# zyang1580/PDA

Measured on AMD Instinct MI355X. Metric: users/sec full-catalogue top-K@50 (eval), higher is better.
Workload: dtype f32; 1 GPU; C3: synthetic 1000000 users x 200000 items, d=128, PDA condition ((elu+1)*pop^0.22) head, masked top-K@50; ranks_seen=1

## Files before the change

__graft_entry__.py:

```python
import os
import subprocess
import sys

ROOT = os.path.dirname(os.path.abspath(__file__))
if ROOT not in sys.path:
    sys.path.insert(0, ROOT)


def build() -> None:
    subprocess.check_call(["make", "-C", os.path.join(ROOT, "pda_amd", "csrc"), "-j4"])
    subprocess.check_call(["make", "-C", os.path.join(ROOT, "oracle")])
    import pda_amd
    from pda_amd import _lib
    _lib.load()


def smoke() -> None:
    import numpy as np
    import torch
    from oracle import c_oracle, pda_oracle as po
    from pda_amd import ops

    assert torch.cuda.is_available(), "smoke() needs a GPU"
    dev = torch.device("cuda:0")
    rng = np.random.default_rng(2021)
    nU, nI, d, B, K = 700, 3000, 64, 512, 50
    U = (rng.standard_normal((nU, d)) * 0.1).astype(np.float32)
    I = (rng.standard_normal((nI, d)) * 0.1).astype(np.float32)
    pop = rng.uniform(0, 1, nI).astype(np.float32) ** 0.22
    hist = [np.unique(rng.integers(0, nI, rng.integers(0, 40))) for _ in range(nU)]
    users = np.arange(nU, dtype=np.int32)
    indptr = np.zeros(nU + 1, dtype=np.int64)
    indptr[1:] = np.cumsum([len(h) for h in hist])
    indices = np.concatenate(hist).astype(np.int32)

    h = ops.HistoryCSR(torch.from_numpy(indptr).to(dev), torch.from_numpy(indices).to(dev), by_user=True)
    idx, val = ops.recommend_topk(torch.from_numpy(U).to(dev), torch.from_numpy(I).to(dev),
                                  torch.from_numpy(users).to(dev), K, ops.HEAD_POP,
                                  torch.from_numpy(pop).to(dev), h)
    ridx, rval, sc = c_oracle.score_topk(U, I, users, K, 1, pop, indptr, indices, order=1, want_scores=True)
    np.testing.assert_allclose(val.cpu().numpy(), rval, rtol=2e-6, atol=1e-6)
    got = idx.cpu().numpy()
    agree = (got == ridx).mean()
    top = np.sort(np.where(np.isfinite(sc), sc, -np.inf), axis=1)[:, ::-1][:, :K + 1]
    gapped = np.min(top[:, :-1] - top[:, 1:], axis=1) > 1e-5
    assert gapped.sum() >= nU // 2, "smoke data should be mostly tie-free"
    np.testing.assert_array_equal(got[gapped], ridx[gapped])
    for r in np.nonzero(~gapped)[0]:
        for a, b in zip(got[r], ridx[r]):
            assert a == b or abs(sc[r, a] - sc[r, b]) <= 1e-5, (r, a, b)

    Ut, It = torch.from_numpy(U).to(dev), torch.from_numpy(I).to(dev)
    us = rng.permutation(nU)[:B].astype(np.int32)
    ps = rng.integers(0, nI, B).astype(np.int32)
    ng = rng.integers(0, nI, B).astype(np.int32)
    pp = pop[ps]
    pn = pop[ng]
    loss = torch.zeros(3, device=dev)
    ops.bpr_step(Ut, It, *(torch.from_numpy(x).to(dev) for x in (us, ps, ng, pp, pn)), regs=1e-2, reg_div=B,
                 lr=0.05, mode=ops.UPD_SGD_FUSED, loss_acc=loss)
    U1, I1, _, ref_loss = po.train_step(U, I, us, ps, ng, pp, pn, 1e-2, B, 0.05, optimizer="sgd")
    np.testing.assert_allclose(loss.cpu().numpy(), np.array(ref_loss), rtol=1e-5, atol=1e-6)
    np.testing.assert_allclose(Ut.cpu().numpy(), U1, atol=1e-6)
    np.testing.assert_allclose(It.cpu().numpy(), I1, atol=1e-6)
    torch.cuda.synchronize()
    print("smoke ok: eval agreement %.5f, loss %s" % (agree, loss.cpu().numpy()))


if __name__ == "__main__":
    build()
    if len(sys.argv) > 1 and sys.argv[1] == "smoke":
        smoke()
```

pda_amd/csrc/pda_score_topk_v4.hip:

```cpp
#include "pda_v4_shared.h"
#include <cstdlib>
#include <type_traits>

using namespace pda_topk;

namespace {

constexpr int kCap4 = 57;
constexpr int kRing4 = 128;
constexpr int kWarmTiles = 4;
constexpr int kMainWaves = 8;
#ifndef PDA_W4_ABL
#define PDA_W4_ABL 0
#endif
#ifndef PDA_V4_ABL
#define PDA_V4_ABL 0
#endif
#ifdef PDA_V4_PROF
__device__ unsigned long long pda_prof4[24];
#define PROF_T0(v) const long long v = __builtin_readcyclecounter()
#define PROF_T1(v, slot) prof[slot] += (unsigned long long)(__builtin_readcyclecounter() - v)
#define PROF_INC(slot, x) prof[slot] += (unsigned long long)(x)
#define PROF_FLUSH(first, last) do { if (lane == 0) for (int pq = (first); pq <= (last); ++pq) atomicAdd(&pda_prof4[pq], prof[pq]); } while (0)
#else
#define PROF_T0(v) do {} while (0)
#define PROF_T1(v, slot) do {} while (0)
#define PROF_INC(slot, x) do {} while (0)
#define PROF_FLUSH(first, last) do {} while (0)
#endif
constexpr unsigned kSpinMax = 1u << 26;


struct Args4 {
    const void* U;
    const void* I;
    const float* pop;
    const int32_t* users;
    const int64_t* hist_indptr;
    const int32_t* hist_indices;
    uint64_t* out_keys;
    const unsigned char* rows;
    const float* sufA;
    const float* sufB;
    const int* pos_of;
    unsigned* stats;
    uint64_t* lists_ws;
    int32_t* regroup_ws;
    float* pred_ws;
    const int32_t* row_perm;
    const uint32_t* hmask_ws;
    const uint32_t* bloom;
    const int* prep_hdr;
    const float* seed;
    int n_users_blk, item_offset, n_items_local, hist_row_mode, K, n_splits, n_tiles;
    int warm_tiles;
    int warm_sorted;
    uint64_t* handover;
    const unsigned char* rows5;
    const float* meta5;
    const unsigned char* ufrag;
    const float* unorm;
    int prep_hdr_pop;
    int warm_final;
    int warm_shared;
    float* seed_out;
    const int* n_users_dev;
    int lists_empty;
};


template <int D, bool BF>
__global__ void __launch_bounds__(256) prep4_kernel(const void* __restrict__ I, const float* __restrict__ pop, const int* __restrict__ order,
                                                    int n, int n_pad, unsigned char* __restrict__ rows, int* __restrict__ pos_of,
                                                    int* __restrict__ hdr, unsigned char* __restrict__ rows5, int* __restrict__ meta5, u32x4* __restrict__ pinfo,
                                                    int f16img) {
    constexpr int TPR = D / 8, RB = row_bytes(D);
    const int pos = blockIdx.x * (256 / TPR) + threadIdx.x / TPR, e = threadIdx.x % TPR;
    if (pos >= n_pad) return;
    unsigned char* rp = rows + (size_t)pos * RB;
    float ss = 0.f, popv = 1.0f, rs = 0.f;
    int src = -1;
    if (pos < n) {
        src = pos;
        if (order) {
            src = order[pos];
            if (src < 0 || src >= n) { if (e == 0) atomicOr(hdr, 1); src = 0; }
            else if (e == 0 && atomicExch(&pos_of[src], pos) != -1) atomicOr(hdr, 1);
        } else if (e == 0) {
            pos_of[pos] = pos;
        }
        if (pop) popv = pop[src];
        const f32x4 a = pda_load4<BF>(I, (size_t)src * D + 8 * e);
        const f32x4 b = pda_load4<BF>(I, (size_t)src * D + 8 * e + 4);
        u32x4 hq, lq;
        split8(a, b, hq, lq);
        *reinterpret_cast<u32x4*>(rp + 16 * e) = hq;
#pragma unroll
        for (int k = 0; k < 4; ++k) ss += a[k] * a[k] + b[k] * b[k];
        {
            const float pv = pop ? ((popv == popv) ? popv : 0.f) : 1.0f;
            f32x4 as = a, bs = b;
#pragma unroll
            for (int k = 0; k < 4; ++k) { as[k] *= pv; bs[k] *= pv; }
            u32x4 hs, ls;
            if (f16img) {
                hs = pack_half8(as, bs, rs);
            } else {
                split8(as, bs, hs, ls);
#pragma unroll
                for (int k = 0; k < 4; ++k) {
                    const float r0 = as[k] - __uint_as_float((k & 1) ? (hs[k >> 1] & 0xFFFF0000u) : (hs[k >> 1] << 16));
                    const float r1 = bs[k] - __uint_as_float((k & 1) ? (hs[2 + (k >> 1)] & 0xFFFF0000u) : (hs[2 + (k >> 1)] << 16));
                    rs += r0 * r0 + r1 * r1;
                }
            }
            const int r5 = pos & 31;
            const int sw = D >= 128 ? (r5 & 15) : ((r5 >> 1) & 7);
            *reinterpret_cast<u32x4*>(rows5 + (size_t)(pos >> 5) * (64 * D) + r5 * (2 * D) + ((e ^ sw) << 4)) = hs;
        }
    } else {
        const u32x4 z = {0u, 0u, 0u, 0u};
        *reinterpret_cast<u32x4*>(rp + 16 * e) = z;
        {
            const int r5 = pos & 31;
            const int sw = D >= 128 ? (r5 & 15) : ((r5 >> 1) & 7);
            *reinterpret_cast<u32x4*>(rows5 + (size_t)(pos >> 5) * (64 * D) + r5 * (2 * D) + ((e ^ sw) << 4)) = z;
        }
    }
#pragma unroll
    for (int o = TPR / 2; o > 0; o >>= 1) { ss += __shfl_xor(ss, o, 64); rs += __shfl_xor(rs, o, 64); }
    if (e == 0) {
        const float v = sqrtf(ss) * 1.0009765625f * 1.0001f;
        const float rv = sqrtf(rs) * 1.0009765625f * 1.0001f;
        {
            if (pos < n) {
                const float pv = pop ? ((popv == popv) ? popv : 0.f) : 1.0f;
                atomicMax(&meta5[4 * (pos >> 5)], __float_as_int(pop ? pv : 0.f));
                atomicMax(&meta5[4 * (pos >> 5) + 1], __float_as_int(pv * v * 1.000001f));
                atomicMax(&meta5[4 * (pos >> 5) + 2], __float_as_int(rv));
            }
        }
        uint32_t p1 = 0x3F80u, p2 = 0, p3 = 0, k1 = 0, k2 = 0;
        if (pop) {
            const float ip = (popv > 0.f) ? fminf((1.0f / popv) * 0.9999995f, 1.0e6f) : 1.0e6f;
            bf16_split3(ip, p1, p2, p3);
            k1 = 0x3F80u;
            k2 = bf16_up(8.0e-6f);
            if (!(popv == popv)) k1 = 0xFF61u;
        } else {
            k1 = bf16_up(8.0e-6f);
// ... 1594 lines not shown
    w.lists = al(pda_score_topk_workspace_bytes(n_users_blk));
    size_t b = w.lists;
    if (lists_in_hbm4(d)) {
        const size_t ut = 1024;
        b += ((size_t)n_users_blk + ut - 1) / ut * (size_t)n_splits * ut * kCap4 * 8 + 256;
    }
    w.bloom = al(b);
    w.hmask = al(w.bloom + (size_t)n_users_blk * 128);
    w.regroup = al(w.hmask + ((size_t)n_users_blk + kUserTile - 1) / kUserTile * (size_t)n_splits * kUserTile * 2 * kWarmTiles * 4);
    w.handover = al(w.regroup + (1024 + 4 * (size_t)n_users_blk) * 4);
    w.total = w.handover + (size_t)n_splits * (size_t)n_users_blk * kCap4 * 8;
    w.ufrag = al(w.total);
    w.unorm = w.ufrag;
    {
        const size_t n_pad = ((size_t)n_users_blk + kUT5 - 1) / kUT5 * kUT5;
        w.unorm = w.ufrag + al(n_pad * 2 * (size_t)d);
        w.total = w.unorm + al(n_pad * 4);
    }
    w.seed = w.total;
    w.total = w.seed + al((size_t)n_users_blk * 4);
    return w;
}
extern "C" size_t pda_score_topk4_workspace_bytes(int n_users_blk, int n_items_local, int d, int n_splits) {
    if (n_users_blk <= 0 || n_items_local <= 0 || (d != 64 && d != 128 && d != 256)) return 0;
    if (n_splits <= 0) n_splits = pda_score_topk4_auto_splits(n_users_blk, n_items_local, d);
    return ws4_layout(n_users_blk, d, n_splits).total;
}

int run_score4(const void* U, const void* I_shard, bool bf16, const void* prep, const float* pop_shard, const int32_t* users,
               int n_users_blk, int item_offset, int n_items_local, int d, const int64_t* hist_indptr, const int32_t* hist_indices,
               int hist_row_mode, int K, int head, int early_stop, int n_splits, uint64_t* out_keys, void* workspace, hipStream_t s,
               int phase = 3, const float* seed = nullptr, int warm_tiles = 0, const int* n_users_dev = nullptr) {
    if (!U || !I_shard || !prep || !users || !out_keys || !workspace) return PDA_ERR_ARG;
    if (n_users_blk <= 0 || n_items_local <= 0 || item_offset < 0) return PDA_ERR_ARG;
    if (K < 1 || K > PDA_MAX_K) return PDA_ERR_ARG;
    if (early_stop < 0 || (early_stop & ~0x7FF) != 0) return PDA_ERR_ARG;
    const bool warm_per_split = (early_stop & PDA_SWEEP_WARM_PER_SPLIT) != 0;
    int geometry = (early_stop & PDA_SWEEP_HUGE) ? 4 : (early_stop & PDA_SWEEP_MANY_CANDIDATES) ? 3 : 0;
    if (warm_tiles == 0) warm_tiles = (early_stop >> 4) & 7;
    early_stop &= 1;
    if (head != PDA_HEAD_RAW && head != PDA_HEAD_POP) return PDA_ERR_ARG;
    if (head == PDA_HEAD_POP && !pop_shard) return PDA_ERR_ARG;
    if (hist_indptr && !hist_indices) return PDA_ERR_ARG;
    if (d != 64 && d != 128 && d != 256) return PDA_ERR_UNSUPPORTED;
    if (K > kCap4 - 3) return PDA_ERR_UNSUPPORTED;
    if ((uint64_t)n_items_local > (1ull << 26)) return PDA_ERR_UNSUPPORTED;
    if (warm_tiles < 0 || warm_tiles > kWarmTiles) return PDA_ERR_ARG;
#ifndef PDA_V4_WARM_DEFAULT
#define PDA_V4_WARM_DEFAULT kWarmTiles
#endif
    if (warm_tiles == 0) warm_tiles = d <= 128 ? PDA_V4_WARM_DEFAULT : kWarmTiles;
    const bool from_empty = phase == 4;
    if (from_empty) {
        if (seed == nullptr) return PDA_ERR_ARG;
        phase = 2;
        warm_tiles = 0;
    } else if (phase < 1 || phase > 3) {
        return PDA_ERR_ARG;
    }
    if (n_splits <= 0) n_splits = pda_score_topk4_auto_splits(n_users_blk, n_items_local, d);
    const Prep4Layout L = prep4_layout(n_items_local, d);
    const unsigned char* pb = reinterpret_cast<const unsigned char*>(prep);
    if (((phase & 1) || from_empty) && hipMemsetAsync(workspace, 0, pda_score_topk_workspace_bytes(n_users_blk), s) != hipSuccess) return PDA_ERR_LAUNCH;
    const Ws4 W = ws4_layout(n_users_blk, d, n_splits);
    unsigned char* wsb = reinterpret_cast<unsigned char*>(workspace);
    const float* sA = reinterpret_cast<const float*>(pb + (head == PDA_HEAD_POP ? L.sufA : L.sufB));
    const float* sB = reinterpret_cast<const float*>(pb + (head == PDA_HEAD_POP ? L.sufB : L.sufR));
    Args4 g{U, I_shard, pop_shard, users, hist_indptr, hist_indices, out_keys, pb + L.rows,
            early_stop ? sA : nullptr, early_stop ? sB : nullptr, reinterpret_cast<const int*>(pb + L.pos_of),
            reinterpret_cast<unsigned*>(workspace), reinterpret_cast<uint64_t*>(wsb + W.lists), nullptr, nullptr, nullptr, nullptr, nullptr, reinterpret_cast<const int*>(pb + L.hdr), seed, n_users_blk, item_offset, n_items_local, hist_row_mode, K, n_splits, L.n_tiles, warm_tiles,
#ifdef PDA_V4_WARM_SORTED
            1, nullptr, pb + L.rows5, reinterpret_cast<const float*>(pb + L.meta5), nullptr, nullptr, 0};
#else
            (phase == 1 || (L.n_tiles + n_splits - 1) / n_splits <= warm_tiles) ? 1 : 0, nullptr,
            pb + L.rows5, reinterpret_cast<const float*>(pb + L.meta5), nullptr, nullptr, 0};
#endif
    if (phase == 3 && !g.warm_sorted && PDA_V4_HANDOVER_WS) g.handover = reinterpret_cast<uint64_t*>(wsb + W.handover);
    g.ufrag = wsb + W.ufrag;
    g.unorm = reinterpret_cast<const float*>(wsb + W.unorm);
    g.prep_hdr_pop = (head == PDA_HEAD_POP && pop_shard != nullptr) ? 1 : 0;
    g.warm_final = (geometry >= 4 && phase == 3 && g.handover != nullptr && g.prep_hdr_pop && !early_stop) ? 1 : 0;
    g.lists_empty = from_empty ? 1 : 0;
    g.n_users_dev = n_users_dev;
    if (phase == 3 && n_splits > 1 && seed == nullptr && !warm_per_split && L.n_tiles > n_splits * warm_tiles) {
        g.warm_shared = 1;
        g.seed_out = reinterpret_cast<float*>(wsb + W.seed);
    }
    if (hist_indptr && (phase & 2)) {
        uint32_t* bloom = reinterpret_cast<uint32_t*>(wsb + W.bloom);
        hipLaunchKernelGGL(hist_bloom4_kernel, dim3((unsigned)((n_users_blk + 31) / 32)), dim3(256), 0, s, users, hist_indptr, hist_indices,
                           hist_row_mode, n_users_blk, bloom, reinterpret_cast<const int*>(pb + L.hdr), head == PDA_HEAD_POP ? 1 : 0);
        PDA_CHECK_LAUNCH();
        g.bloom = bloom;
    }
    if (hist_indptr && (phase & 1) && n_users_blk >= 98304) {
        uint32_t* hm = reinterpret_cast<uint32_t*>(wsb + W.hmask);
        const int utiles = (n_users_blk + kUserTile - 1) / kUserTile;
        Args4 gm = g;
        if (g.warm_shared) {
            gm.n_splits = 1;
            gm.warm_shared = 0;
        }
        hipLaunchKernelGGL(warm_mask4_kernel, dim3((unsigned)(utiles * gm.n_splits)), dim3(kThreads), 0, s, gm, hm);
        PDA_CHECK_LAUNCH();
        g.hmask_ws = hm;
    }
#ifndef PDA_V4_REGROUP_MIN
#define PDA_V4_REGROUP_MIN 98304
#endif
    if (early_stop && (phase & 2) && n_splits == 1 && n_users_blk >= PDA_V4_REGROUP_MIN) {
        g.regroup_ws = reinterpret_cast<int32_t*>(wsb + W.regroup);
        if (phase & 1) g.pred_ws = reinterpret_cast<float*>(g.regroup_ws + 1024 + 2 * (size_t)n_users_blk);
    }
    if (head == PDA_HEAD_RAW) {
        g.sufA = early_stop ? reinterpret_cast<const float*>(pb + L.sufA) : nullptr;
        g.sufB = early_stop ? reinterpret_cast<const float*>(pb + L.sufR) : nullptr;
    }
#define PDA_V4_(DD, BFV) (head == PDA_HEAD_POP ? launch4<DD, PDA_HEAD_POP, BFV>(g, phase, s, geometry) : launch4<DD, PDA_HEAD_RAW, BFV>(g, phase, s, geometry))
    switch (d) {
        case 64: return bf16 ? PDA_V4_(64, true) : PDA_V4_(64, false);
        case 128: return bf16 ? PDA_V4_(128, true) : PDA_V4_(128, false);
        case 256: return bf16 ? PDA_V4_(256, true) : PDA_V4_(256, false);
        default: return PDA_ERR_UNSUPPORTED;
    }
#undef PDA_V4_
}

__global__ void __launch_bounds__(256) kth_value_kernel(const uint64_t* __restrict__ keys, int S, int n_users, int K, int pos, float* __restrict__ out) {
    const int u = blockIdx.x * 256 + threadIdx.x;
    if (u >= n_users) return;
    float best = -INFINITY;
    for (int sp = 0; sp < S; ++sp) {
        const uint64_t k = keys[((size_t)sp * n_users + u) * K + pos];
        if (k != 0ull) best = fmaxf(best, pda_key_val(k));
    }
    out[u] = best;
}

__global__ void __launch_bounds__(256) seed_refine_kernel(const uint64_t* __restrict__ keys, int S, int n_users, int K, float* __restrict__ lo,
                                                          float* __restrict__ hi, float* __restrict__ mid, int32_t* __restrict__ counts, int mode) {
    const int u = blockIdx.x * 256 + threadIdx.x;
    if (u >= n_users) return;
    float l = lo[u], h = hi[u];
    if (mode >= 1) {
        if (counts[u] >= K) l = mid[u];
        else h = mid[u];
        lo[u] = l;
        hi[u] = h;
    }
    if (mode <= 1) {
        const bool open = l > -INFINITY && h < INFINITY && h > l;
        const float m = open ? l + 0.5f * (h - l) : l;
        int c = 0;
        for (int sp = 0; sp < S; ++sp) {
            const uint64_t* row = keys + ((size_t)sp * n_users + u) * K;
            for (int q = 0; q < K; ++q) {
                const uint64_t k = row[q];
                if (k == 0ull || pda_key_val(k) < m) break;
                ++c;
            }
        }
        mid[u] = m;
        counts[u] = c;
    }
}

// ... 193 lines not shown
```

pda_amd/csrc/pda_v5_sweep.h:

```cpp
#pragma once
#ifdef PDA_V6_LOOP_HEADER
#include PDA_V6_LOOP_HEADER
#else
#include "pda_v6_loop_asm.h"
#endif

#ifdef PDA_V5_LOG
__device__ unsigned pda_v5_log[1 << 18];
#define V5LOG(kind, a, b) do { if (lane == 0) { const unsigned i_ = atomicAdd(&pda_v5_log[0], 1u); if (i_ < (1u << 16) - 1u) { \
    pda_v5_log[4 * i_ + 4] = ((unsigned)blockIdx.x << 8) | (unsigned)wave; pda_v5_log[4 * i_ + 5] = (kind); pda_v5_log[4 * i_ + 6] = (a); pda_v5_log[4 * i_ + 7] = (b); } } } while (0)
#else
#define V5LOG(kind, a, b) do {} while (0)
#endif
constexpr int kRing5 = 192;



template <int D, bool BF, bool S16, int UPW>
__global__ void __launch_bounds__(256, 1) sweep5_kernel(Args4 g) {
    [[maybe_unused]] constexpr int HB = half_bytes5(D);
    static_assert(slot_bytes5(D) == Loop6<D, 8>::kSlotBytes, "one LDS image for all loops");
    static_assert(S16, "the loop on v_mfma_f32_32x32x16_bf16 (round 4's first form: 9.16 against 8.07 ms, profiles/README.md) left with round 5; the parameter keeps the kernel's name");
    static_assert((D <= 128 && UPW == 256) || (D == 256 && UPW == 128), "users per wave: 256, or (d = 256) 128 -- 8 blocks x 8 k-steps = 256 AGPRs, one 512-user workgroup per CU");
    constexpr int NK = D / 32, UBW = 16, NU = UPW / UBW;
    constexpr int SS = slot_bytes5(D), UT = 4 * UPW, CAPL = kCap4, RB4 = row_bytes(D);
    constexpr int LPC = D / 32, CPP = 64 / LPC;
    constexpr float kEps5 = BF ? 4.0234375e-3f : 8.046875e-3f;
    extern __shared__ __attribute__((aligned(16))) unsigned char smem[];
    unsigned char* tiles = smem;
    int* cntl = reinterpret_cast<int*>(smem + kNSlot5 * SS);
    float* taul = reinterpret_cast<float*>(cntl + UT);
    uint64_t* crings = reinterpret_cast<uint64_t*>(taul + UT);
    unsigned* sync = reinterpret_cast<unsigned*>(crings + 4 * kRing5);
    unsigned* s_uns = sync + 8;
    unsigned* touched = sync + 40;
    const int tid = threadIdx.x, lane = tid & 63;
    const int wave = __builtin_amdgcn_readfirstlane(tid >> 6);
    const int split = blockIdx.x % g.n_splits, utile = blockIdx.x / g.n_splits;
    uint64_t* lists = g.handover != nullptr ? g.handover + ((size_t)split * g.n_users_blk + (size_t)utile * UT) * kCap4
                                            : g.lists_ws + (size_t)blockIdx.x * UT * CAPL;
    const int K = g.K;
    const int nt = split_tiles(g.n_tiles, split, g.n_splits);
    const int wt = warm_tiles_of(g, split);
    const bool starts_empty = g.lists_empty || (g.warm_shared && split > 0);
    const bool warm_final = g.warm_final && !starts_empty;
    const int n_it = max(0, nt - wt);
    const unsigned hend = 2u * (unsigned)n_it;
    if (tid < 72) sync[tid] = (tid < 8 || tid >= 40 || warm_final || starts_empty) ? 0u : 0xFFFFFFFFu;
    if (tid == 0 && blockIdx.x == 0) g.stats[4] = (4u << 28) | (4u << 8) | (1u << 13) | ((BF ? 1u : 0u) << 14) | (unsigned)(D >> 6);
    if (starts_empty) {
        for (int rr = tid; rr < UT; rr += 256) {
            cntl[rr] = 0;
            taul[rr] = utile * UT + rr < g.n_users_blk ? -INFINITY : INFINITY;
        }
        __builtin_amdgcn_fence(__ATOMIC_RELEASE, "workgroup");
    } else if (warm_final) {
        for (int rr = tid; rr < UT; rr += 256) {
            const int rb = utile * UT + rr;
            int c = 0;
            float tau = INFINITY;
            if (rb < g.n_users_blk) {
                const uint64_t kl = lists[(size_t)rr * CAPL + (K - 1)];
                c = K;
                tau = pda_unordf((uint32_t)(kl >> 32));
                if (kl == 0ull) {
                    tau = -INFINITY;
                    for (c = 0; c < K - 1 && lists[(size_t)rr * CAPL + c] != 0ull; ++c) {}
                }
            }
            cntl[rr] = c;
            taul[rr] = tau;
        }
        __builtin_amdgcn_fence(__ATOMIC_RELEASE, "workgroup");
    } else
    {
        constexpr int NW = 4, PB = 8;
        for (int r0 = wave; r0 < UT; r0 += PB * NW) {
            uint64_t keyv[PB];
#pragma unroll
            for (int q = 0; q < PB; ++q) {
                const int rr = r0 + q * NW, rb = utile * UT + rr;
                keyv[q] = (rr >= UT || rb >= g.n_users_blk) ? 0ull
                          : g.handover != nullptr ? (lane < kCap4 ? g.handover[((size_t)split * g.n_users_blk + rb) * kCap4 + lane] : 0ull)
                          : (lane < K ? g.out_keys[((size_t)split * g.n_users_blk + rb) * K + lane] : 0ull);
            }
#pragma unroll
            for (int q = 0; q < PB; ++q) {
                const int rr = r0 + q * NW;
                if (rr >= UT) break;
                const int rb = utile * UT + rr;
                const uint64_t key = keyv[q];
                const int c = __popcll(__ballot(key != 0ull));
                if (g.handover == nullptr && lane < K) lists[(size_t)rr * CAPL + lane] = key;
                uint32_t mn = key != 0ull ? (uint32_t)(key >> 32) : 0xFFFFFFFFu;
#pragma unroll
                for (int o = 32; o >= 1; o >>= 1) mn = min(mn, (uint32_t)__shfl_xor((int)mn, o, 64));
                if (lane == 0) {
                    cntl[rr] = c;
                    taul[rr] = rb < g.n_users_blk ? (c >= K ? pda_unordf(mn) : -INFINITY) : INFINITY;
                }
            }
        }
        __builtin_amdgcn_fence(__ATOMIC_RELEASE, "workgroup");
    }
    __syncthreads();

    unsigned n_cand = 0;
    if (hend > 0) {
        const int row0 = wave * UPW;
        const int j = lane & (UBW - 1), hh = lane / UBW;
        const unsigned lane16 = (unsigned)lane * 16u;
        const unsigned char* my_ufrag = g.ufrag + ((size_t)utile * 4 + wave) * (size_t)(NU * NK * 1024);
        float eu = 0.f, seedv[NU];
#pragma unroll
        for (int u = 0; u < NU; ++u) {
            const int rb = utile * UT + row0 + UBW * u + j;
            eu = fmaxf(eu, rb < g.n_users_blk ? g.unorm[rb] : 0.f);
            seedv[u] = (g.seed != nullptr && rb < g.n_users_blk) ? g.seed[rb] : -INFINITY;
        }
#pragma unroll
        for (int o = 32; o >= 1; o >>= 1) eu = fmaxf(eu, __shfl_xor(eu, o, 64));
        eu = __int_as_float(__builtin_amdgcn_readfirstlane(__float_as_int(eu * (kEps5 * 1.001f))));
        const unsigned ring_lds = (unsigned)(size_t)(__attribute__((address_space(3))) unsigned char*)tiles;
        const unsigned flags_lds = (unsigned)(size_t)(__attribute__((address_space(3))) unsigned char*)reinterpret_cast<unsigned char*>(sync);
        uint64_t* my_ring = crings + wave * kRing5;
        unsigned ring_n = 0;
        const unsigned t0 = (unsigned)(split + wt * g.n_splits);
        const size_t img = (size_t)g.rows5, meta = (size_t)g.meta5;
        const bool hist_on = g.hist_indptr != nullptr;

        auto thr_of = [&](int u) __attribute__((always_inline)) -> float {
            const float tq = fmaxf(taul[row0 + UBW * u + j], seedv[u]);
            float tf = (tq == INFINITY || tq == -INFINITY) ? tq : tq - fabsf(tq) * 1.52587890625e-5f - 1e-30f;
            return fminf(fmaxf(tf, -1.0e30f), 1.0e30f);
        };
        auto rescore_ring = [&]() __attribute__((always_inline)) {
            const int q = lane % LPC, ci = lane / LPC;
            for (unsigned base = 0; base < ring_n; base += CPP) {
                const bool have = base + (unsigned)ci < ring_n;
                const uint64_t e = have ? my_ring[base + ci] : 0ull;
                const int row = (int)(e >> 32);
                const unsigned pos = (unsigned)e;
                bool valid = have && pos < (unsigned)g.n_items_local;
                const unsigned char* tail = g.rows + (size_t)(valid ? pos : 0u) * RB4 + 2 * D + 32;
                const float pv = *reinterpret_cast<const float*>(tail);
                const int loc = *reinterpret_cast<const int*>(tail + 4);
                const int rb = utile * UT + row0 + row;
                valid = valid && rb < g.n_users_blk;
                const int uid = valid ? g.users[rb] : 0;
                const float c_sd = (g.seed != nullptr && valid) ? g.seed[rb] : -INFINITY;
                const float c_tau = taul[row0 + (valid ? row : 0)];
                f32x4 uu[8], ii[8];
                const size_t ub = (size_t)uid * D + q * (LPC == 8 ? 32 : 8), ib = (size_t)(valid ? loc : 0) * D + q * (LPC == 8 ? 32 : 8);
#pragma unroll
                for (int c = 0; c < 8; ++c) {
                    const int off = LPC == 8 ? 4 * c : 8 * LPC * (c >> 1) + 4 * (c & 1);
                    uu[c] = pda_load4<BF>(g.U, ub + off);
                    ii[c] = pda_load4<BF>(g.I, ib + off);
                }
                long long hb = 0, he = 0;
                if (hist_on && valid) {
                    const int64_t hr = g.hist_row_mode == PDA_HIST_BY_USER_ID ? (int64_t)uid : (int64_t)rb;
                    hb = g.hist_indptr[hr];
                    he = g.hist_indptr[hr + 1];
                }
                auto fma8 = [&](float acc, int cq) __attribute__((always_inline)) -> float {
#pragma unroll
                    for (int sidx = 0; sidx < 4; ++sidx) {
                        acc = __builtin_fmaf(uu[2 * cq][sidx], ii[2 * cq][sidx], acc);
                        acc = __builtin_fmaf(uu[2 * cq + 1][sidx], ii[2 * cq + 1][sidx], acc);
                    }
                    return acc;
                };
                float o = 0.f, o_other = 0.f;
                if constexpr (LPC == 8) {
                    float c0 = 0.f, c1 = 0.f, o0 = 0.f, o1 = 0.f;
#pragma unroll
                    for (int ph = 0; ph < LPC; ++ph) {
                        o0 = c0;
                        o1 = c1;
#pragma unroll
                        for (int cc = 0; cc < 4; ++cc) {
#pragma unroll
                            for (int sidx = 0; sidx < 4; ++sidx) {
                                if (cc & 1) {
                                    o1 = __builtin_fmaf(uu[2 * cc][sidx], ii[2 * cc][sidx], o1);
                                    o1 = __builtin_fmaf(uu[2 * cc + 1][sidx], ii[2 * cc + 1][sidx], o1);
                                } else {
                                    o0 = __builtin_fmaf(uu[2 * cc][sidx], ii[2 * cc][sidx], o0);
                                    o0 = __builtin_fmaf(uu[2 * cc + 1][sidx], ii[2 * cc + 1][sidx], o0);
                                }
                            }
                        }
                        if (ph < LPC - 1) {
                            const float r0 = __shfl_up(o0, 1, 64), r1 = __shfl_up(o1, 1, 64);
                            if (q == ph + 1) {
                                c0 = r0;
                                c1 = r1;
                            }
                        }
                    }
                    o = o1;
                    o_other = o0;
                } else if constexpr (LPC == 4) {
// ... 6 lines not shown
                        const float a = fma8(o, cq);
                        const float a_sw = swap2(a);
                        const float b = fma8(hi ? a_sw : o, cq);
                        const float b_sw = swap2(b);
                        o = hi ? b : b_sw;
                    }
                } else {
                    static_assert(LPC == 2, "d = 64");
#pragma unroll
                    for (int cq = 0; cq < 4; ++cq) o = fma8(o, cq);
                }
                const float o0 = LPC == 8 ? o_other : __int_as_float(__builtin_amdgcn_mov_dpp(__float_as_int(o), 0xB1, 0xF, 0xF, true));
                float sc = o0 + o;
                sc = (sc > 0.0f ? sc + 1.0f : __expf(sc)) * pv;
                const float tt = (valid && q == LPC - 1) ? sc : -INFINITY;
                const int item = g.item_offset + loc;
                bool p = valid && q == LPC - 1 && (tt >= fmaxf(c_tau, c_sd));
                if (hist_on && p) {
                    long long lo = hb, hi2 = he;
                    while (lo < hi2) {
                        const long long mid = (lo + hi2) >> 1;
                        if (g.hist_indices[mid] < item) lo = mid + 1; else hi2 = mid;
                    }
                    if (lo < he && g.hist_indices[lo] == item) p = false;
                }
                const uint64_t key = pda_pack_key(tt, (uint32_t)item);
                if (p) atomicOr(&touched[(row0 + row) >> 5], 1u << ((row0 + row) & 31));
                append_keys<CAPL, true>(p, row0 + row, tt, key, lists, cntl, taul, row0, UPW, K, lane, s_uns);
            }
            n_cand += ring_n;
            ring_n = 0;
        };
        auto extract = [&](unsigned ft) __attribute__((always_inline)) {
            const unsigned T = t0 + (ft >> 1) * (unsigned)g.n_splits;
            const unsigned pos0 = T * 64u + (ft & 1u) * 32u;
            const float2 mt = *reinterpret_cast<const float2*>(g.meta5 + 4 * (size_t)(2u * T + (ft & 1u)));
            const float ct = __builtin_fmaf(eu, mt.y, mt.x);
            const unsigned char* tb = tiles + (ft & (kNSlot5 - 1)) * SS + j * (2 * D);
            auto item_of = [&](int r) __attribute__((always_inline)) -> unsigned {
                return 16u * (r >> 2) + 4u * hh + (r & 3);
            };
            constexpr int NR = 8;
            u32x4 af[2 * NK];
#pragma unroll
            for (int ib = 0; ib < 2; ++ib)
#pragma unroll
                for (int k = 0; k < NK; ++k) af[ib * NK + k] = *reinterpret_cast<const u32x4*>(tb + ib * 16 * (2 * D) + (((4 * k + hh) ^ swz5<D>(j)) << 4));
            for (int u = 0; u < NU; ++u) {
                const float tl = thr_of(u);
                const bool clampy = mt.x > tl;
                uint32_t m = 0;
#pragma unroll
                for (int ib = 0; ib < 2; ++ib) {
                    f32x4 acc = {0.f, 0.f, 0.f, 0.f};
#pragma unroll
                    for (int k = 0; k < NK; ++k) {
                        const u32x4 bf = *reinterpret_cast<const u32x4*>(my_ufrag + (((size_t)u * NK + k) * 64 + lane) * 16);
                        acc = __builtin_amdgcn_mfma_f32_16x16x32_bf16(__builtin_bit_cast(bf16x8, af[ib * NK + k]), __builtin_bit_cast(bf16x8, bf), acc, 0, 0, 0);
                    }
#pragma unroll
                    for (int r = 0; r < 4; ++r) m |= (acc[r] + ct > tl) ? (1u << (4 * ib + r)) : 0u;
                }
                if (__any(clampy)) {
#pragma unroll
                    for (int r = 0; r < NR; ++r) {
                        const unsigned pp = pos0 + item_of(r);
                        const float pi = clampy ? *reinterpret_cast<const float*>(g.rows + (size_t)pp * RB4 + 2 * D + 32) : 0.f;
                        m |= (clampy && pi > tl) ? (1u << r) : 0u;
                    }
                }
                while (__any(m != 0u)) {
                    if (ring_n + 64u > (unsigned)kRing5) rescore_ring();
                    const bool act = m != 0u;
                    const int r = __builtin_ctz(m | 0x10000u);
                    m &= ~(1u << r);
                    const uint64_t pm = __ballot(act);
                    const unsigned slot = ring_n + (unsigned)__builtin_amdgcn_mbcnt_hi((uint32_t)(pm >> 32), __builtin_amdgcn_mbcnt_lo((uint32_t)pm, 0));
                    if (act) my_ring[slot] = ((uint64_t)(unsigned)(UBW * u + j) << 32) | (uint64_t)(pos0 + item_of(r));
                    ring_n += (unsigned)__popcll(pm);
                }
            }
        };

        unsigned h = 0, issued = 0, n_entries = 0;
        bool hend_ok = true;
        if ((ring_lds & (D == 256 ? 511u : 255u)) != 0u) { if (lane == 0) g.stats[0] = 6u; hend_ok = false; }
        for (unsigned guard = 0; hend_ok && guard < 2u * hend + 8u; ++guard) {
            ++n_entries;
            float thr[NU];
#pragma unroll
            for (int u = 0; u < NU; ++u) thr[u] = thr_of(u);
            unsigned reason = 0;
            float tmin = thr[0];
#pragma unroll
            for (int u = 1; u < NU; ++u) tmin = fminf(tmin, thr[u]);
#pragma unroll
            for (int o = 32; o >= 1; o >>= 1) tmin = fminf(tmin, __shfl_xor(tmin, o, 64));
            tmin = __int_as_float(__builtin_amdgcn_readfirstlane(__float_as_int(tmin)));
            Loop6<D, NU>::run(h, issued, reason, hend, ring_lds, flags_lds, 1024u * (unsigned)wave, t0, (unsigned)g.n_splits,
                              (unsigned)img, (unsigned)(img >> 32), (unsigned)meta, (unsigned)(meta >> 32), eu, tmin, my_ufrag, thr, lane16);
            V5LOG(reason, h, issued);
            if (reason == 0u) break;
            if (reason != 1u) { if (lane == 0) g.stats[0] = 5u; break; }
#ifdef PDA_V5_LOG
            for (unsigned tq = (h >= 2u ? h - 2u : 0u); tq <= h && tq < hend; ++tq) {
                const unsigned Tq = t0 + (tq >> 1) * (unsigned)g.n_splits;
                const unsigned char* gsrc = g.rows5 + ((size_t)(2u * Tq + (tq & 1u))) * HB;
                const unsigned char* lsrc = tiles + (tq & (kNSlot5 - 1)) * SS;
                unsigned pieces = 0;
                for (int i = 0; i < HB / 1024; ++i) {
                    const u32x4 a4 = *reinterpret_cast<const u32x4*>(gsrc + i * 1024 + lane * 16);
                    const u32x4 b4 = *reinterpret_cast<const u32x4*>(lsrc + i * 1024 + lane * 16);
                    if (__ballot(((a4[0] ^ b4[0]) | (a4[1] ^ b4[1]) | (a4[2] ^ b4[2]) | (a4[3] ^ b4[3])) != 0u) != 0ull) pieces |= 1u << i;
                }
                if (pieces != 0u) V5LOG(13u, (tq << 8) | (h - tq), pieces);
            }
#endif
            [[maybe_unused]] const unsigned before = ring_n + n_cand;
            if (h >= 2u && h - 2u < hend) extract(h - 2u);
            if (h >= 1u && h - 1u < hend) extract(h - 1u);
            V5LOG(10u, h, ring_n + n_cand - before);
            if (ring_n >= (unsigned)CPP) rescore_ring();
        }
        if (ring_n > 0u) rescore_ring();
        if (lane == 0) atomicAdd(g.stats + 1, n_cand);
        if (lane == 0) atomicAdd(g.stats + 5, n_entries);
        if (lane == 0 && wave == 0) atomicAdd(reinterpret_cast<unsigned long long*>(g.stats + 2), (unsigned long long)(2 * n_it * (UT / kUserTile)));
    }
    __builtin_amdgcn_fence(__ATOMIC_ACQ_REL, "workgroup");
    __syncthreads();
    {
        constexpr int EB = 8;
        uint64_t* scr = crings + wave * kRing5;
        auto emit_row = [&](int rb, int cnt, uint64_t kraw) __attribute__((always_inline)) {
            const int c = min(__builtin_amdgcn_readfirstlane(cnt), CAPL);
            const uint64_t key = lane < c ? kraw : (uint64_t)(63 - lane);
            scr[lane] = key;
            pda_wave_sync();
            int rank = 0;
            for (int jj = 0; jj < c; jj += 4) {
                const uint64_t k0 = scr[jj], k1 = scr[jj + 1], k2 = scr[jj + 2], k3 = scr[jj + 3];
                rank += ((k0 > key) ? 1 : 0) + ((k1 > key) ? 1 : 0) + ((k2 > key) ? 1 : 0) + ((k3 > key) ? 1 : 0);
            }
            pda_wave_sync();
            uint64_t* orow = g.out_keys + ((size_t)split * g.n_users_blk + rb) * K;
            if (lane < c && rank < K) orow[rank] = key;
            if (lane >= c && lane < K) orow[lane] = 0ull;
        };
        if (warm_final) {
            for (int w = 0; w < UPW / 32; ++w) {
                unsigned m = touched[wave * (UPW / 32) + w];
                while (m != 0u) {
                    const int b = __builtin_ctz(m);
                    m &= m - 1u;
                    const int rr = wave * UPW + 32 * w + b;
                    emit_row(utile * UT + rr, cntl[rr], lists[(size_t)rr * CAPL + (lane < CAPL ? lane : CAPL - 1)]);
                }
            }
        } else if (starts_empty) {
            const int rb0 = utile * UT + wave * UPW, nv = max(0, min(UPW, g.n_users_blk - rb0));
            uint64_t* ob = g.out_keys + ((size_t)split * g.n_users_blk + rb0) * K;
            for (int i = lane; i < nv * K; i += 64) ob[i] = 0ull;
            __builtin_amdgcn_fence(__ATOMIC_RELEASE, "workgroup");
            for (int w = 0; w < UPW / 32; ++w) {
                unsigned m = touched[wave * (UPW / 32) + w];
                while (m != 0u) {
                    const int b = __builtin_ctz(m);
                    m &= m - 1u;
                    const int rr = wave * UPW + 32 * w + b;
                    emit_row(utile * UT + rr, cntl[rr], lists[(size_t)rr * CAPL + (lane < CAPL ? lane : CAPL - 1)]);
                }
            }
        } else {
            for (int i0 = 0; i0 < UPW; i0 += EB) {
                uint64_t kraw[EB];
                int cv[EB];
#pragma unroll
                for (int q = 0; q < EB; ++q) {
                    const int rr = wave * UPW + i0 + q, rb = utile * UT + rr;
                    const bool ok = rb < g.n_users_blk;
                    kraw[q] = ok ? lists[(size_t)rr * CAPL + (lane < CAPL ? lane : CAPL - 1)] : 0ull;
                    cv[q] = ok ? cntl[rr] : 0;
                }
#pragma unroll
                for (int q = 0; q < EB; ++q) {
                    const int rb = utile * UT + wave * UPW + i0 + q;
                    if (rb >= g.n_users_blk) break;
                    emit_row(rb, cv[q], kraw[q]);
                }
            }
        }
    }
}

template <int D, bool BF, bool S16, int UPW>
int launch_sweep5(const Args4& g, hipStream_t stream) {
    constexpr int UT = 4 * UPW;
    constexpr size_t lds = (size_t)kNSlot5 * slot_bytes5(D) + (size_t)UT * 8 + 4 * kRing5 * 8 + 80 * 4 + 64;
    static_assert(UPW == 256 || D == 256 || 2 * lds <= 160 * 1024, "two workgroups per CU");
    static_assert(lds <= 160 * 1024, "LDS per workgroup");
    static int attr_set = 0;
    if (!attr_set) {
        if (hipFuncSetAttribute(reinterpret_cast<const void*>(&sweep5_kernel<D, BF, S16, UPW>), hipFuncAttributeMaxDynamicSharedMemorySize, (int)lds) != hipSuccess)
            return PDA_ERR_LAUNCH;
        attr_set = 1;
    }
    const int utiles = (g.n_users_blk + UT - 1) / UT, n_pad = utiles * UT;
    hipLaunchKernelGGL((uprep5_kernel<D, BF, S16, UPW>), dim3((unsigned)(((size_t)n_pad * (D / 8) + 255) / 256)), dim3(256), 0, stream, g.U, g.users, g.n_users_blk, n_pad,
                       const_cast<unsigned char*>(g.ufrag), const_cast<float*>(g.unorm));
// ... 6 lines not shown
```

pda_amd/ops.py:

```python
from __future__ import annotations

import math
import os
from typing import Optional, Tuple

import ctypes as C

import torch

from . import _lib
from ._lib import (HEAD_POP, HEAD_RAW, HIST_BY_BLOCK_ROW, HIST_BY_USER_ID, UPD_ANY_ORDER, UPD_DENSE_GRAD, UPD_NONE, UPD_USERS_DISTINCT,
                   UPD_SGD_FUSED, check, ptr, stream_ptr)

ADAM_BETA1, ADAM_BETA2, ADAM_EPS = 0.9, 0.999, 1e-8


def _need(t: Optional[torch.Tensor], dtype, name: str, optional=False):
    if t is None:
        if optional:
            return None
        raise ValueError(f"{name} is required")
    if not t.is_cuda:
        raise ValueError(f"{name} must live in HBM (cuda tensor); pda_amd has no CPU path")
    if t.dtype != dtype:
# ... 323 lines not shown
    if pop_shard is not None and pop_shard.numel() != nloc:
        raise ValueError("pop_shard must have one entry per local item row")
    if nloc > (1 << 26):
        raise ValueError("seeded item-sharded evaluation: at most 2^26 item rows per shard")
    if head == HEAD_POP and pop_shard is not None:
        _check_pop(pop_shard)
    if hist is not None and hist.indices.numel() == 0:
        hist = None
    c = SeededCall()
    order = visiting_order(I_shard, pop_shard if head == HEAD_POP else None)
    prep = item_prep4(I_shard, pop_shard if head == HEAD_POP else None, order)
    if n_splits <= 0:
        n_splits = lib.pda_score_topk4_auto_splits(nu, nloc, d)
    c.lib, c.K, c.nu, c.n_splits, c.nloc, c.stats = lib, K, nu, n_splits, nloc, stats
    c.out = torch.empty((n_splits, nu, K), dtype=torch.int64, device=U.device)
    c.ws = torch.empty(lib.pda_score_topk4_workspace_bytes(nu, nloc, d, n_splits), dtype=torch.uint8, device=U.device)
    c.fnp = lib.pda_score_topk4_phase_bf16 if bf else lib.pda_score_topk4_phase_f32
    c.common = (ptr(U), ptr(I_shard), ptr(prep), ptr(pop_shard), ptr(users), nu, item_offset, nloc, d,
                ptr(hist.indptr) if hist else None, ptr(hist.indices) if hist else None, hist.mode if hist else 0, K, head,
                1 | few_candidates_hint(head, True, nu, d), n_splits)
    c.keep = (U, I_shard, prep, pop_shard, users, hist)
    c.wt = int(os.environ.get("PDA_WARM_TILES", "0")) or max(1, 4 // max(1, seed_shards))
    check(c.fnp(*c.common, 1, c.wt, None, ptr(c.out), ptr(c.ws), stream_ptr()), "pda_score_topk4_phase (warm-up)")
    c.bounds = torch.empty((3, nu), dtype=torch.float32, device=U.device)
    m = -(-K // max(1, seed_shards))
    check(lib.pda_topk_seed_bounds(ptr(c.out), n_splits, nu, K, m, ptr(c.bounds), stream_ptr()), "pda_topk_seed_bounds")
    c.n_thr, c.counts = seed_thresholds(seed_shards), None
    return c


def kth_value(keys: torch.Tensor, pos: int) -> torch.Tensor:
    keys = _need(keys, torch.int64, "keys")
    S, nu, K = keys.shape
    out = torch.empty(nu, dtype=torch.float32, device=keys.device)
    check(_lib.load().pda_topk_kth_value(ptr(keys), S, nu, K, int(pos), ptr(out), stream_ptr()), "pda_topk_kth_value")
    return out


def remap_key_items(keys: torch.Tensor, gid: torch.Tensor) -> torch.Tensor:
    keys = _need(keys, torch.int64, "keys")
    gid = _need(gid, torch.int32, "gid")
    check(_lib.load().pda_topk_remap_items(ptr(keys), keys.numel(), ptr(gid), gid.numel(), stream_ptr()), "pda_topk_remap_items")
    return keys


def sweep_from_seed(U, I_shard, users, K, head, pop_shard, hist, item_offset, seed: torch.Tensor, n_splits: int = 0, prune="order",
                    stats: Optional[dict] = None) -> torch.Tensor:
    lib = _lib.load()
    bf = I_shard.dtype == torch.bfloat16
    U = _need(U, torch.bfloat16 if bf else torch.float32, "U")
    I_shard = _need(I_shard, torch.bfloat16 if bf else torch.float32, "I_shard")
    users = _need(users, torch.int32, "users")
    seed = _need(seed, torch.float32, "seed")
    pop_shard = _need(pop_shard, torch.float32, "pop_shard", optional=True)
    nu, nloc, d = users.numel(), I_shard.shape[0], I_shard.shape[1]
    if seed.numel() != nu:
        raise ValueError("seed must have one entry per user of the block")
    if d not in (64, 128, 256) or K > TOPK_K_V4:
        raise ValueError("sweep_from_seed: embed dim 64/128/256 and K <= %d" % TOPK_K_V4)
    if head == HEAD_POP and pop_shard is not None:
        _check_pop(pop_shard)
    if hist is not None and hist.indices.numel() == 0:
        hist = None
    order = visiting_order(I_shard, pop_shard if head == HEAD_POP else None) if prune else None
    prep = item_prep4(I_shard, pop_shard if head == HEAD_POP else None, order)
    if n_splits <= 0:
        n_splits = lib.pda_score_topk4_auto_splits(nu, nloc, d)
        if head == HEAD_POP and prune == "order" and d in (64, 128, 256) and not os.environ.get("PDA_SCORE_LISTS") and pop_shard is not None:
            n_splits = huge_splits(nu, nloc, d) or n_splits
    out = torch.empty((n_splits, nu, K), dtype=torch.int64, device=U.device)
    ws = torch.empty(lib.pda_score_topk4_workspace_bytes(nu, nloc, d, n_splits), dtype=torch.uint8, device=U.device)
    es = (1 if prune is True else 0) | few_candidates_hint(head, prune, nu, d, nloc, n_splits)
    fn = lib.pda_score_topk4_phase_bf16 if bf else lib.pda_score_topk4_phase_f32
    check(fn(ptr(U), ptr(I_shard), ptr(prep), ptr(pop_shard), ptr(users), nu, item_offset, nloc, d,
             ptr(hist.indptr) if hist else None, ptr(hist.indices) if hist else None, hist.mode if hist else 0, K, head, es, n_splits,
             4, 0, ptr(seed), ptr(out), ptr(ws), stream_ptr()), "pda_score_topk4_phase (sweep from a seed)")
    if os.environ.get("PDA_CHECK_SWEEP_ERRORS"):
        err = int(ws[0:4].view(torch.int32)[0])
        if err != 0:
            raise RuntimeError("pda_score_topk4_phase: the sweep reported protocol error %d" % err)
    if stats is not None:
        stats["pairs_rescored"] = ws[4:8].view(torch.int32)
        stats["kernel_id"] = ws[16:20].view(torch.int32)
        stats["error"] = ws[0:4].view(torch.int32)
    return out


def seeded_counts(c: SeededCall) -> Optional[torch.Tensor]:
    if c.n_thr <= 0:
        return None
    c.counts = torch.empty((c.n_thr, c.nu), dtype=torch.int32, device=c.bounds.device)
    check(c.lib.pda_topk_seed_counts(ptr(c.out), c.n_splits, c.nu, c.K, ptr(c.bounds), c.n_thr, ptr(c.counts), stream_ptr()),
          "pda_topk_seed_counts")
    return c.counts


def seeded_finish(c: SeededCall) -> torch.Tensor:
    seed = torch.empty(c.nu, dtype=torch.float32, device=c.bounds.device)
    check(c.lib.pda_topk_seed_pick(ptr(c.bounds), ptr(c.counts), c.n_thr if c.counts is not None else 0, c.nu, c.K, ptr(seed), stream_ptr()),
          "pda_topk_seed_pick")
    check(c.fnp(*c.common, 2, c.wt, ptr(seed), ptr(c.out), ptr(c.ws), stream_ptr()), "pda_score_topk4_phase (sweep)")
    if c.stats is not None:
        c.stats["tiles_scored"] = c.ws[8:16].view(torch.int64)
        c.stats["pairs_rescored"] = c.ws[4:8].view(torch.int32)
        c.stats["tiles_dense"] = ((c.nloc + 31) // 32) * ((c.nu + 127) // 128)
        c.stats["kernel_id"] = c.ws[16:20].view(torch.int32)
        c.stats["error"] = c.ws[0:4].view(torch.int32)
    out, c.keep = c.out, None
    return out


def score_topk_keys(U, I_shard, users, K=50, head=HEAD_RAW, pop_shard=None, hist: Optional[HistoryCSR] = None,
                    item_offset=0, n_splits=0, out: Optional[torch.Tensor] = None, impl: Optional[str] = None,
                    prune=None, stats: Optional[dict] = None, seed_reduce=None, seed_shards: int = 1, seed_sum=None,
                    warm_tiles: int = 0) -> torch.Tensor:
    lib = _lib.load()
    bf = I_shard is not None and I_shard.dtype == torch.bfloat16
    U = _need(U, torch.bfloat16 if bf else torch.float32, "U")
    I_shard = _need(I_shard, torch.bfloat16 if bf else torch.float32, "I_shard")
    users = _need(users, torch.int32, "users")
    pop_shard = _need(pop_shard, torch.float32, "pop_shard", optional=True)
    nu, nloc, d = users.numel(), I_shard.shape[0], I_shard.shape[1]
    if bf:
        if d not in (64, 128, 256) or K > TOPK_CAP_V2 or impl == "v1":
            raise ValueError("bf16 tables: embed dim 64/128/256, K <= %d, no v1 entry point" % TOPK_CAP_V2)
        impl = "v2"
    if U.shape[1] != d:
        raise ValueError("U and I_shard disagree on embed dim")
    if pop_shard is not None and pop_shard.numel() != nloc:
        raise ValueError("pop_shard must have one entry per local item row")
    if head == HEAD_POP and pop_shard is not None:
        _check_pop(pop_shard)
    if hist is not None and hist.indices.numel() == 0:
        hist = None
    n_splits_auto = n_splits <= 0
    out_given = out
    impl = impl or score_impl(d, K, item_offset + nloc)
    if prune is None:
        prune = prune_default(head, d)
    if seed_reduce is not None and seed_exchange_applies(d, K, head, prune, impl):
        if out_given is not None:
            raise ValueError("the seeded sweep allocates its own output")
        c = seeded_begin(U, I_shard, users, K, head, pop_shard, hist, item_offset, n_splits, seed_shards, stats=stats)
        seed_reduce(c.bounds)
        cnt = seeded_counts(c) if seed_sum is not None else None
        if cnt is not None:
            seed_sum(cnt)
        return seeded_finish(c)
    if n_splits_auto and out_given is None and impl == "v2" and funnel_applies(d, K, nu, nloc, head, prune, hist):
        return score_topk_funnel(U, I_shard, users, K, hist, item_offset, stats)
    if n_splits <= 0:
        n_splits = lib.pda_score_topk_auto_splits(nu, nloc)
    if out is None:
        out = torch.empty((n_splits, nu, K), dtype=torch.int64, device=U.device)
    elif out.shape != (n_splits, nu, K) or out.dtype != torch.int64:
        raise ValueError("out must be int64 [n_splits, Bu, K]")
    if impl == "v2" and score_kernel(d, K, nloc, prune, head) == "v4":
        order = visiting_order(I_shard, pop_shard if head == HEAD_POP else None) if prune else None
        prep = item_prep4(I_shard, pop_shard if head == HEAD_POP else None, order)
        forced_env = any(os.environ.get(k) for k in ("PDA_SCORE_LISTS", "PDA_SCORE_KERNEL", "PDA_HUGE_SPLITS"))
        plan = None
        if n_splits_auto and out_given is None and not forced_env and not (head == HEAD_POP and pop_shard is None):
            plan = score_plan(nu, nloc, d, K, head, prune, bf, hist)
            if plan["kernel"] != "v4":
                plan = None
        if plan is not None:
            n_splits = plan["n_splits"]
            out = torch.empty((n_splits, nu, K), dtype=torch.int64, device=U.device)
        elif n_splits_auto and out_given is None:
            n_splits = lib.pda_score_topk4_auto_splits(nu, nloc, d)
            if head == HEAD_POP and prune == "order" and d in (64, 128, 256) and not os.environ.get("PDA_SCORE_LISTS") and pop_shard is not None:
                n_splits = huge_splits(nu, nloc, d) or n_splits
            out = torch.empty((n_splits, nu, K), dtype=torch.int64, device=U.device)
        ws = torch.empty(lib.pda_score_topk4_workspace_bytes(nu, nloc, d, n_splits), dtype=torch.uint8, device=U.device)
        hint = plan["early_stop"] if plan is not None else ((1 if prune is True else 0) | few_candidates_hint(head, prune, nu, d, nloc, n_splits))
        es = hint | ((min(4, max(0, int(warm_tiles))) & 7) << 4)
        if os.environ.get("PDA_WARM_PER_SPLIT"):
            es |= SWEEP_WARM_PER_SPLIT
        fn = lib.pda_score_topk4_bf16 if bf else lib.pda_score_topk4_f32
        check(fn(ptr(U), ptr(I_shard), ptr(prep), ptr(pop_shard), ptr(users), nu, item_offset, nloc, d,
                 ptr(hist.indptr) if hist else None, ptr(hist.indices) if hist else None, hist.mode if hist else 0,
                 K, head, es, n_splits, ptr(out), ptr(ws), stream_ptr()), "pda_score_topk4")
        if os.environ.get("PDA_CHECK_SWEEP_ERRORS"):
            err = int(ws[0:4].view(torch.int32)[0])
            if err != 0:
                raise RuntimeError("pda_score_topk4: the sweep reported protocol error %d" % err)
        if stats is not None:
            stats["tiles_scored"] = ws[8:16].view(torch.int64)
            stats["pairs_rescored"] = ws[4:8].view(torch.int32)
            stats["tiles_dense"] = ((nloc + 31) // 32) * ((nu + 127) // 128)
            stats["kernel_id"] = ws[16:20].view(torch.int32)
            stats["huge_entries"] = ws[20:24].view(torch.int32)
            stats["error"] = ws[0:4].view(torch.int32)
        return out
    if impl == "v2" and prune:
        prep, order = item_prep_ordered(I_shard, pop_shard if head == HEAD_POP else None)
        hist_ord = hist_reordered(hist, prep, order, item_offset, nloc, d) if hist else None
        ws = torch.empty(lib.pda_score_topk_workspace_bytes(nu), dtype=torch.uint8, device=U.device)
        fn = lib.pda_score_topk_ordered_bf16 if bf else lib.pda_score_topk_ordered_f32
        check(fn(ptr(U), ptr(I_shard), ptr(prep), ptr(pop_shard), ptr(users), nu, item_offset,
                                             nloc, d, ptr(hist.indptr) if hist else None,
                                             ptr(hist.indices) if hist else None, ptr(hist_ord), hist.mode if hist else 0,
                                             K, head, 0 if prune == "order" else 1, n_splits, ptr(out), ptr(ws), stream_ptr()),
              "pda_score_topk_ordered")
        if stats is not None:
            stats["tiles_scored"] = ws[8:16].view(torch.int64)
            stats["pairs_rescored"] = ws[4:8].view(torch.int32)
            stats["tiles_dense"] = ((nloc + 31) // 32) * ((nu + 127) // 128)
            stats["kernel_id"] = ws[16:20].view(torch.int32)
        return out
    if impl == "v2":
        prep = item_prep(I_shard)
        ws = torch.empty(lib.pda_score_topk_workspace_bytes(nu), dtype=torch.uint8, device=U.device)
        fn = lib.pda_score_topk_bf16 if bf else lib.pda_score_topk_prepped_f32
        check(fn(ptr(U), ptr(I_shard), ptr(prep), ptr(pop_shard), ptr(users), nu, item_offset,
                                             nloc, d, ptr(hist.indptr) if hist else None,
                                             ptr(hist.indices) if hist else None, hist.mode if hist else 0, K, head,
                                             n_splits, ptr(out), ptr(ws), stream_ptr()), "pda_score_topk_prepped_f32")
        return out
    check(lib.pda_score_topk_f32(ptr(U), ptr(I_shard), ptr(pop_shard), ptr(users), nu, item_offset, nloc, d,
                                 ptr(hist.indptr) if hist else None, ptr(hist.indices) if hist else None,
                                 hist.mode if hist else 0, K, head, n_splits, ptr(out), stream_ptr()),
          "pda_score_topk_f32")
    return out


FUNNEL_MIN_USERS = 1
FUNNEL_MIN_ITEMS = 4096
FUNNEL_BLOCK_ROW_MAX_USERS = 16384
FUNNEL_SMALL_ITEMS, FUNNEL_SMALL_MAX_USERS = 20000, 16384
_FUNNEL_ORDER = {}


def funnel_order(I_shard: torch.Tensor) -> torch.Tensor:
    key = (I_shard.shape[0], str(I_shard.device))
    o = _FUNNEL_ORDER.get(key)
    if o is None:
        g = torch.Generator(device="cpu").manual_seed(0x5EED + I_shard.shape[0])
        o = torch.randperm(I_shard.shape[0], generator=g).to(torch.int32).to(I_shard.device)
        _FUNNEL_ORDER[key] = o
    return o


FUNNEL_WORKSPACE_BUDGET = 24 << 30


def funnel_applies(d: int, K: int, nu: int, nloc: int, head: int, prune, hist: Optional[HistoryCSR]) -> bool:
    can = head == HEAD_RAW and d in (64, 128, 256) and K <= TOPK_K_V4 and 4096 <= nloc <= (1 << 26) and prune is not True \
        and (hist is None or hist.mode == HIST_BY_USER_ID or nu <= FUNNEL_BLOCK_ROW_MAX_USERS)
    forced = os.environ.get("PDA_SCORE_FUNNEL", "")
    if forced == "0" or not can:
        return False
    if forced == "1":
        return True
    return nu >= FUNNEL_MIN_USERS and nloc >= FUNNEL_MIN_ITEMS and (nloc >= FUNNEL_SMALL_ITEMS or nu <= FUNNEL_SMALL_MAX_USERS) \
        and not os.environ.get("PDA_SCORE_KERNEL") and not os.environ.get("PDA_SCORE_LISTS") \
        and _lib.load().pda_score_topk7_workspace_bytes(nu, nloc, d) <= FUNNEL_WORKSPACE_BUDGET


def score_topk_funnel(U, I_shard, users, K=50, hist: Optional[HistoryCSR] = None, item_offset=0, stats: Optional[dict] = None) -> torch.Tensor:
    lib = _lib.load()
    bf = I_shard.dtype == torch.bfloat16
    U = _need(U, torch.bfloat16 if bf else torch.float32, "U")
    I_shard = _need(I_shard, torch.bfloat16 if bf else torch.float32, "I_shard")
    users = _need(users, torch.int32, "users")
    nu, nloc, d = users.numel(), I_shard.shape[0], I_shard.shape[1]
    if hist is not None and hist.indices.numel() == 0:
        hist = None
    prep = item_prep7(I_shard, funnel_order(I_shard))
    out = torch.empty((1, nu, K), dtype=torch.int64, device=U.device)
    nbytes = lib.pda_score_topk7_workspace_bytes(nu, nloc, d)
    if nbytes == 0:
        raise ValueError("the funnel: embed dim 64 / 128 / 256")
    ws = torch.empty(nbytes, dtype=torch.uint8, device=U.device)
    fn = lib.pda_score_topk7_bf16 if bf else lib.pda_score_topk7_f32
# ... 805 lines not shown
```

Measured before the change: 30.39 million users/s.

## Finish sweep with a check-free loop once tail bounds prove no candidates remain

Each wave publishes its minimum threshold and maximum user norm to LDS, and after a block barrier the workgroup binary-searches the popularity-ordered suffix bounds (tailA/tailB) for the first half-tile whose bound falls below the workgroup threshold. The guarded sweep then only runs up to that limit, and the remaining half-tiles go through a new Loop6Free path. The intent is to avoid per-tile threshold checks and candidate extraction on tiles that can no longer contribute. The cost is an extra __syncthreads and a binary search on every loop entry, plus the risk of mishandling the ring buffer or the tail indices.

```diff
diff --git a/__graft_entry__.py b/__graft_entry__.py
--- a/__graft_entry__.py
+++ b/__graft_entry__.py
@@ -8,7 +8,7 @@
 
 
 def build() -> None:
-    subprocess.check_call(["make", "-C", os.path.join(ROOT, "pda_amd", "csrc"), "-j4"])
+    subprocess.check_call(["make", "-C", os.path.join(ROOT, "pda_amd", "csrc"), "-j4", "PYTHON=" + sys.executable])
     subprocess.check_call(["make", "-C", os.path.join(ROOT, "oracle")])
     import pda_amd
     from pda_amd import _lib
diff --git a/pda_amd/csrc/pda_score_topk_v4.hip b/pda_amd/csrc/pda_score_topk_v4.hip
--- a/pda_amd/csrc/pda_score_topk_v4.hip
+++ b/pda_amd/csrc/pda_score_topk_v4.hip
@@ -66,6 +66,8 @@
     float* seed_out;
     const int* n_users_dev;
     int lists_empty;
+    const float* tailA;
+    const float* tailB;
 };
 
 
@@ -1826,6 +1828,10 @@
     g.warm_final = (geometry >= 4 && phase == 3 && g.handover != nullptr && g.prep_hdr_pop && !early_stop) ? 1 : 0;
     g.lists_empty = from_empty ? 1 : 0;
     g.n_users_dev = n_users_dev;
+    if (g.prep_hdr_pop) {
+        g.tailA = reinterpret_cast<const float*>(pb + L.sufA);
+        g.tailB = reinterpret_cast<const float*>(pb + L.sufB);
+    }
     if (phase == 3 && n_splits > 1 && seed == nullptr && !warm_per_split && L.n_tiles > n_splits * warm_tiles) {
         g.warm_shared = 1;
         g.seed_out = reinterpret_cast<float*>(wsb + W.seed);
diff --git a/pda_amd/csrc/pda_v5_sweep.h b/pda_amd/csrc/pda_v5_sweep.h
--- a/pda_amd/csrc/pda_v5_sweep.h
+++ b/pda_amd/csrc/pda_v5_sweep.h
@@ -4,6 +4,7 @@
 #else
 #include "pda_v6_loop_asm.h"
 #endif
+#include "pda_v6_free_asm.h"
 
 #ifdef PDA_V5_LOG
 __device__ unsigned pda_v5_log[1 << 18];
@@ -120,6 +121,7 @@
         }
 #pragma unroll
         for (int o = 32; o >= 1; o >>= 1) eu = fmaxf(eu, __shfl_xor(eu, o, 64));
+        const float numax = eu;
         eu = __int_as_float(__builtin_amdgcn_readfirstlane(__float_as_int(eu * (kEps5 * 1.001f))));
         const unsigned ring_lds = (unsigned)(size_t)(__attribute__((address_space(3))) unsigned char*)tiles;
         const unsigned flags_lds = (unsigned)(size_t)(__attribute__((address_space(3))) unsigned char*)reinterpret_cast<unsigned char*>(sync);
@@ -292,11 +294,26 @@
             }
         };
 
-        unsigned h = 0, issued = 0, n_entries = 0;
+        auto decided = [&](float tw, float nw, unsigned h_now) __attribute__((always_inline)) -> unsigned {
+#ifdef PDA_V5_NO_FREE
+            return hend;
+#else
+            if (g.tailA == nullptr || !(tw > -1.0e30f)) return hend;
+            int lo = (int)(h_now >> 1), hi = n_it;
+            while (lo < hi) {
+                const int mid = (lo + hi) >> 1;
+                const size_t T = (size_t)t0 + (size_t)mid * (size_t)g.n_splits;
+                if (__builtin_fmaf(nw, g.tailB[T], g.tailA[T]) * 1.000002f < tw) hi = mid; else lo = mid + 1;
+            }
+            return 2u * (unsigned)lo;
+#endif
+        };
+        float* xch = reinterpret_cast<float*>(sync + 72);
+        unsigned h = 0, issued = 0, n_entries = 0, n_free = 0;
+        unsigned hlim = hend;
         bool hend_ok = true;
         if ((ring_lds & (D == 256 ? 511u : 255u)) != 0u) { if (lane == 0) g.stats[0] = 6u; hend_ok = false; }
         for (unsigned guard = 0; hend_ok && guard < 2u * hend + 8u; ++guard) {
-            ++n_entries;
             float thr[NU];
 #pragma unroll
             for (int u = 0; u < NU; ++u) thr[u] = thr_of(u);
@@ -307,13 +324,34 @@
 #pragma unroll
             for (int o = 32; o >= 1; o >>= 1) tmin = fminf(tmin, __shfl_xor(tmin, o, 64));
             tmin = __int_as_float(__builtin_amdgcn_readfirstlane(__float_as_int(tmin)));
-            Loop6<D, NU>::run(h, issued, reason, hend, ring_lds, flags_lds, 1024u * (unsigned)wave, t0, (unsigned)g.n_splits,
+            if (lane == 0) { xch[wave] = tmin; xch[4 + wave] = numax; }
+            __syncthreads();
+            const float tw = __int_as_float(__builtin_amdgcn_readfirstlane(__float_as_int(fminf(fminf(xch[0], xch[1]), fminf(xch[2], xch[3])))));
+            const float nw = __int_as_float(__builtin_amdgcn_readfirstlane(__float_as_int(fmaxf(fmaxf(xch[4], xch[5]), fmaxf(xch[6], xch[7])))));
+            const unsigned hf = decided(tw, nw, h);
+            if (h >= min(hlim, hf)) {
+                if (h > hlim) h = hlim;
+                if (issued > hlim) issued = hlim;
+                if (h < hend) {
+                    ++n_entries;
+                    n_free = hend - h;
+                    Loop6Free<D, NU>::run(h, issued, hend, ring_lds, 1024u * (unsigned)wave, t0, (unsigned)g.n_splits, (unsigned)img, (unsigned)(img >> 32), my_ufrag, lane16);
+                    V5LOG(14u, h, n_free);
+                }
+                break;
+            }
+            hlim = min(hlim, hf);
+            ++n_entries;
+            Loop6<D, NU>::run(h, issued, reason, hlim, ring_lds, flags_lds, 1024u * (unsigned)wave, t0, (unsigned)g.n_splits,
                               (unsigned)img, (unsigned)(img >> 32), (unsigned)meta, (unsigned)(meta >> 32), eu, tmin, my_ufrag, thr, lane16);
             V5LOG(reason, h, issued);
-            if (reason == 0u) break;
+            if (reason == 0u) {
+                if (hlim == hend) break;
+                continue;
+            }
             if (reason != 1u) { if (lane == 0) g.stats[0] = 5u; break; }
 #ifdef PDA_V5_LOG
-            for (unsigned tq = (h >= 2u ? h - 2u : 0u); tq <= h && tq < hend; ++tq) {
+            for (unsigned tq = (h >= 2u ? h - 2u : 0u); tq <= h && tq < hlim; ++tq) {
                 const unsigned Tq = t0 + (tq >> 1) * (unsigned)g.n_splits;
                 const unsigned char* gsrc = g.rows5 + ((size_t)(2u * Tq + (tq & 1u))) * HB;
                 const unsigned char* lsrc = tiles + (tq & (kNSlot5 - 1)) * SS;
@@ -327,14 +365,15 @@
             }
 #endif
             [[maybe_unused]] const unsigned before = ring_n + n_cand;
-            if (h >= 2u && h - 2u < hend) extract(h - 2u);
-            if (h >= 1u && h - 1u < hend) extract(h - 1u);
+            if (h >= 2u && h - 2u < hlim) extract(h - 2u);
+            if (h >= 1u && h - 1u < hlim) extract(h - 1u);
             V5LOG(10u, h, ring_n + n_cand - before);
             if (ring_n >= (unsigned)CPP) rescore_ring();
         }
         if (ring_n > 0u) rescore_ring();
         if (lane == 0) atomicAdd(g.stats + 1, n_cand);
         if (lane == 0) atomicAdd(g.stats + 5, n_entries);
+        if (lane == 0 && wave == 0 && n_free > 0u) atomicAdd(g.stats + 7, n_free);
         if (lane == 0 && wave == 0) atomicAdd(reinterpret_cast<unsigned long long*>(g.stats + 2), (unsigned long long)(2 * n_it * (UT / kUserTile)));
     }
     __builtin_amdgcn_fence(__ATOMIC_ACQ_REL, "workgroup");
diff --git a/pda_amd/ops.py b/pda_amd/ops.py
--- a/pda_amd/ops.py
+++ b/pda_amd/ops.py
@@ -429,6 +429,8 @@
     if stats is not None:
         stats["pairs_rescored"] = ws[4:8].view(torch.int32)
         stats["kernel_id"] = ws[16:20].view(torch.int32)
+        stats["huge_entries"] = ws[20:24].view(torch.int32)
+        stats["huge_free_halftiles"] = ws[28:32].view(torch.int32)
         stats["error"] = ws[0:4].view(torch.int32)
     return out
 
@@ -538,6 +540,7 @@
             stats["tiles_dense"] = ((nloc + 31) // 32) * ((nu + 127) // 128)
             stats["kernel_id"] = ws[16:20].view(torch.int32)
             stats["huge_entries"] = ws[20:24].view(torch.int32)
+            stats["huge_free_halftiles"] = ws[28:32].view(torch.int32)
             stats["error"] = ws[0:4].view(torch.int32)
         return out
     if impl == "v2" and prune:
```

Result: faster. 32.19 million users/s, median of 6 (+5.9%).
